# knelk/enerf

Hardware: AMD Instinct MI355X
Metric: train_rays_per_sec (higher is better)
Workload: dtype f32

## Files before the change

### enerf_amd/_lib.py

```python
import ctypes
import os

_HERE = os.path.dirname(os.path.abspath(__file__))
LIB_PATH = os.path.join(_HERE, "lib", "libenerf_hip.so")
if os.environ.get("ENERF_LIB_PATH"):
    LIB_PATH = os.environ["ENERF_LIB_PATH"]

_c = ctypes
_vp, _u32, _f32, _int, _sz = _c.c_void_p, _c.c_uint32, _c.c_float, _c.c_int, _c.c_size_t

SIGNATURES = {
    "enerf_near_far_from_aabb": [_vp, _vp, _vp, _u32, _f32, _vp, _vp, _vp],
    "enerf_polar_from_ray": [_vp, _vp, _f32, _u32, _vp, _vp],
    "enerf_morton3D": [_vp, _u32, _vp, _vp],
    "enerf_morton3D_invert": [_vp, _u32, _vp, _vp],
    "enerf_packbits": [_vp, _u32, _f32, _vp, _vp],
    "enerf_march_rays_train": [_vp, _vp, _vp, _f32, _f32, _u32, _u32, _u32, _u32, _u32, _vp, _vp, _vp, _vp, _vp,
                               _vp, _vp, _u32, _vp],
    "enerf_march_fuse_near_far": [_vp, _f32],
    "enerf_march_mirror_count": [_vp],
    "enerf_march_rays_train_ex": [_vp, _vp, _vp, _f32, _f32, _u32, _u32, _u32, _u32, _u32, _vp, _vp, _vp, _vp, _vp,
                                  _vp, _vp, _u32, _u32, _vp],
    "enerf_march_rays_train_count": [_vp, _vp, _vp, _f32, _f32, _u32, _u32, _u32, _u32, _vp, _vp, _vp, _vp, _u32, _u32,
                                     _vp],
# ... 31 lines not shown
    "enerf_mlp32_io16": [_int],
    "enerf_grid_adam_from_records_ex": [_vp, _vp, _vp, _vp, _vp, _u32, _u32, _f32, _f32, _f32, _f32, _u32, _u32, _vp, _vp,
                                        _vp, _vp, _vp, _vp, _vp, _vp],
    "enerf_grid_adam_from_records": [_vp, _vp, _vp, _vp, _vp, _u32, _u32, _f32, _f32, _f32, _f32, _u32, _vp],
    "enerf_sh_encode_forward": [_vp, _vp, _u32, _u32, _u32, _int, _vp, _int, _vp],
    "enerf_sh_encode_backward": [_vp, _vp, _u32, _u32, _u32, _vp, _vp, _int, _vp],
    "enerf_ffmlp_forward": [_vp, _vp, _u32, _u32, _u32, _u32, _u32, _u32, _u32, _vp, _vp, _int, _vp],
    "enerf_ffmlp_inference": [_vp, _vp, _u32, _u32, _u32, _u32, _u32, _u32, _u32, _vp, _vp, _int, _vp],
    "enerf_ffmlp_backward": [_vp, _vp, _vp, _vp, _u32, _u32, _u32, _u32, _u32, _u32, _u32, _int, _vp, _vp, _vp,
                             _int, _vp],
    "enerf_ffnerf_inference": [_vp, _vp, _vp, _vp, _u32, _int, _vp, _vp, _vp],
    "enerf_mlp32_forward": [_vp, _vp, _u32, _u32, _u32, _u32, _u32, _u32, _vp, _vp, _u32, _u32, _vp, _vp],
    "enerf_mlp32_forward_p": [_vp, _vp, _u32, _u32, _u32, _u32, _u32, _u32, _u32, _u32, _vp, _vp, _u32, _u32, _vp, _vp,
                              _vp],
    "enerf_mlp32_backward_p": [_vp, _vp, _vp, _vp, _u32, _u32, _u32, _vp, _u32, _u32, _u32, _u32, _u32, _vp, _vp, _u32,
                               _u32, _vp, _u32, _vp, _vp, _u32, _vp],
    "enerf_mlp32_forward_sh": [_vp, _vp, _u32, _u32, _u32, _u32, _u32, _u32, _vp, _vp, _u32, _u32, _vp, _vp, _vp],
    "enerf_mlp32_backward": [_vp, _vp, _vp, _vp, _u32, _u32, _u32, _u32, _u32, _vp, _vp, _vp, _u32, _u32, _vp, _u32, _vp, _vp,
                             _u32, _vp],
    "enerf_sh_encode_forward_strided": [_vp, _vp, _u32, _u32, _u32, _vp],
    "enerf_debug_grid_level_mask": [_u32],
    "enerf_debug_sweep_route": [_u32, _u32],
    "enerf_debug_sweep_schedule": [_u32, _u32, _u32, _vp, _u32],
    "enerf_debug_mlp32_wgrad_blocks": [_u32],
    "enerf_debug_mlp32_grid_caps": [_u32, _u32],
    "enerf_debug_march_wave_max_rays": [_u32],
    "enerf_debug_march_bg_blocks": [_u32],
    "enerf_debug_march_clip": [_int],
    "enerf_march_rays_use_box": [_int],
    "enerf_grid_owner_range": [ctypes.c_uint64, ctypes.c_uint64, _f32],
    "enerf_ffmlp_recompute": [_int],
    "enerf_amp_begin": [_vp, _vp, _vp, _vp],
    "enerf_amp_end": [_f32, _f32, _int, _vp],
    "enerf_amp_cancel": [],
    "enerf_debug_march_thread_min_rays": [_u32],
    "enerf_event_loss_fwd_bwd": [_vp, _vp, _vp, _u32, _u32, _u32, _f32, _f32, _f32, _vp, _vp, _vp, _vp, _vp],
    "enerf_event_pair_rays": [_vp, _vp, _vp, _vp, _u32, _vp, _vp, _u32, _u32, _vp, _vp, _vp, _vp, _u32, _f32, _f32, _f32,
                              _f32, _vp, _vp, _vp, _vp, _vp, _vp, _vp, _vp, _vp],
    "enerf_occupied_box_update": [_vp, _u32, _u32, _f32, _vp],
    "enerf_debug_mlp32_fused_backward": [_int],
    "enerf_mlp32_precision": [_int],
    "enerf_mlp32_recompute": [_int],
    "enerf_debug_grid_bwd_binned": [_u32, _u32],
    "enerf_density_grid_cells": [_vp, _u32, _u32, _f32, _u32, _c.c_uint64, _vp, _vp, _vp],
    "enerf_mark_untrained_grid": [_vp, _u32, _u32, _f32, _f32, _f32, _f32, _u32, _u32, _f32, _vp, _vp],
    "enerf_density_grid_update": [_vp, _vp, _u32, _u32, _u32, _f32, _f32, _f32, _vp, _vp, _vp, _u32, _vp, _vp],
# ... 206 lines not shown
```

### enerf_amd/csrc/common.h

```cpp
#pragma once
#include <hip/hip_runtime.h>
#include <stdint.h>
#include <stdio.h>

#include "../../include/enerf_hip.h"

namespace enerf {

constexpr int kWave = 64;

void set_error(const char* fmt, ...);

inline int check_hip(hipError_t e, const char* what) {
    if (e != hipSuccess) {
        set_error("%s: %s", what, hipGetErrorString(e));
        return (int)e;
    }
    return 0;
}

#define ENERF_BADARG(...)            \
    do {                             \
        enerf::set_error(__VA_ARGS__); \
        return ENERF_E_BADARG;       \
// ... 9 lines not shown
    int id;
    hipStream_t s;
    void* slot;
    bool ext;
    ProfScope(int kernel_id, hipStream_t stream, bool ext = false);
    ~ProfScope();
    hipEvent_t start() const;
    hipEvent_t stop() const;
    void units(double n) const;
};

struct AmpState {
    const float* scale;
    uint32_t* found_inf;
    const uint32_t* skipped;
};
AmpState amp_state();

void* workspace(int slot, size_t bytes);
uint64_t workspace_generation();
uint32_t num_cus();
int workspace_family_enter(int family, hipStream_t s);
int single_device_guard(const char* what);
enum { WS_SCAN = 0, WS_COMPACT = 1, WS_FFMLP = 2, WS_GRIDBWD = 3, WS_MARCH = 4, WS_DENSITY = 5, WS_MLP32_DEFER = 6, WS_AABB = 7, WS_AABB_CALL = 8, WS_FFMLP_W = 9, WS_NERF_FRAGS = 10, WS_NERF_PART = 11, WS_MARCH2 = 12, WS_SLOTS = 13 };

__host__ __device__ inline uint32_t div_up(uint32_t a, uint32_t b) { return (a + b - 1) / b; }

struct SplitJob {
    const float* src[5];
    const uint32_t* map;
    uint32_t* out;
    uint32_t threads;
};
struct ValidRows {
    const int32_t* count;
    uint32_t base, cap;
};
int grid_encode_forward(const float* inputs, const void* embeddings, const int32_t* offsets, void* outputs, uint32_t B,
                        uint32_t D, uint32_t C, uint32_t L, float S, uint32_t H, int calc_grad_inputs, void* dy_dx,
                        uint32_t gridtype, int dtype, int out_layout, float in_add, float in_mul, enerf_stream_t stream,
                        const ValidRows& grid_valid_rows, const SplitJob* job = nullptr, bool* carried = nullptr);
int grid_encode_backward(const void* grad, const float* inputs, const int32_t* offsets, void* grad_embeddings, uint32_t B,
                         uint32_t D, uint32_t C, uint32_t L, float S, uint32_t H, int calc_grad_inputs, const void* dy_dx,
                         void* grad_inputs, uint32_t gridtype, int dtype, int grad_layout, float in_add, float in_mul,
                         uint32_t flags, uint32_t reserve_B, enerf_stream_t stream, const ValidRows& grid_valid_rows);
struct MlpCall {
    ValidRows rows;
// ... 130 lines not shown
```

### enerf_amd/csrc/density_update.hip

```cpp

#include "common.h"
#include "sweep_points.h"

using namespace enerf;

namespace {

__device__ __forceinline__ uint32_t morton3(uint32_t x, uint32_t y, uint32_t z) { return sweep_morton3(x, y, z); }
__device__ __forceinline__ uint32_t compact_bits(uint32_t x) {
    x = x & 0x49249249;
    x = (x | (x >> 2)) & 0xc30c30c3;
    x = (x | (x >> 4)) & 0x0f00f00f;
    x = (x | (x >> 8)) & 0xff0000ff;
    x = (x | (x >> 16)) & 0x0000ffff;
    return x;
}

__global__ void __launch_bounds__(256) k_cells_full(Cascades cs, uint32_t C, uint32_t H, uint32_t logH, uint64_t seed,
                                                    int32_t* __restrict__ indices, float* __restrict__ xyzs) {
    const uint32_t H3 = H * H * H;
    const uint32_t p = blockIdx.x * blockDim.x + threadIdx.x;
    if (p >= C * H3) return;
    const uint32_t cas = p / H3, cell = p - cas * H3;
    const uint32_t x = cell & (H - 1), y = (cell >> logH) & (H - 1), z = cell >> (2 * logH);
// ... 197 lines not shown
    }
    __syncthreads();
    const uint32_t nh = heavy_n < 64u ? heavy_n : 64u;
    for (uint32_t e = 0; e < nh; e++) {
        const uint32_t key = heavy[e][0], c = heavy[e][1], at = heavy[e][2];
        for (uint32_t j = threadIdx.x; j < c; j += 256) out[at + j] = key;
    }
}

__global__ void __launch_bounds__(256) k_cells_from_keys(Cascades cs, uint32_t P, uint32_t H, uint32_t bits,
                                                         uint64_t seed, const uint32_t* __restrict__ keys,
                                                         int32_t* __restrict__ indices, float* __restrict__ xyzs) {
    const uint32_t p = blockIdx.x * blockDim.x + threadIdx.x;
    if (p >= P) return;
    const uint32_t key = keys[p];
    const uint32_t idx = key & ((1u << bits) - 1), cas = key >> bits;
    indices[p] = (int32_t)idx;
    cell_position(cs, cas, H, compact_bits(idx), compact_bits(idx >> 1), compact_bits(idx >> 2), rand4(seed, p),
                  xyzs + (size_t)p * 3);
}

__global__ void __launch_bounds__(256) k_tmp_scatter(const int32_t* __restrict__ indices, const float* __restrict__ sigmas,
                                                     uint32_t n_per_cas, uint32_t P, uint32_t H3, float scale,
                                                     float* __restrict__ tmp, uint32_t H, uint32_t logH) {
    const uint32_t p = blockIdx.x * blockDim.x + threadIdx.x;
    if (p >= P) return;
    const uint32_t cas = p / n_per_cas;
    uint32_t idx;
    if (indices) {
        idx = (uint32_t)indices[p];
    } else {
        const uint32_t cell = p - cas * n_per_cas;
        idx = morton3(cell & (H - 1), (cell >> logH) & (H - 1), cell >> (2 * logH));
    }
    tmp[(size_t)cas * H3 + idx] = sigmas[p] * scale;
}

constexpr uint32_t kSumSlots = 16, kSumStride = 16, kSumBytes = kSumSlots * kSumStride * 8;

__global__ void k_zero_sums(double* __restrict__ sum) { sum[threadIdx.x] = 0.0; }

__device__ __forceinline__ float ema1(float g, float t, float decay, float& acc) {
    if (g >= 0.0f && t >= 0.0f) g = fmaxf(g * decay, t);
    acc += fmaxf(g, 0.0f);
    return g;
}

__global__ void __launch_bounds__(256) k_ema_mean(float* __restrict__ grid, const float* __restrict__ tmp, uint32_t total4,
                                                  float decay, double* __restrict__ sum) {
    __shared__ float wsum[4];
    float acc = 0.0f;
    for (uint32_t i = blockIdx.x * blockDim.x + threadIdx.x; i < total4; i += gridDim.x * blockDim.x) {
        float4 g = reinterpret_cast<float4*>(grid)[i];
        const float4 t = reinterpret_cast<const float4*>(tmp)[i];
        g.x = ema1(g.x, t.x, decay, acc); g.y = ema1(g.y, t.y, decay, acc);
        g.z = ema1(g.z, t.z, decay, acc); g.w = ema1(g.w, t.w, decay, acc);
        reinterpret_cast<float4*>(grid)[i] = g;
    }
    for (int o = 32; o > 0; o >>= 1) acc += __shfl_down(acc, o, 64);
    if (lane_id() == 0) wsum[threadIdx.x >> 6] = acc;
    __syncthreads();
    if (threadIdx.x == 0)
        atomicAdd(sum + (blockIdx.x % kSumSlots) * kSumStride, (double)((wsum[0] + wsum[1]) + (wsum[2] + wsum[3])));
}

__global__ void __launch_bounds__(256) k_packbits_mean(const float* __restrict__ grid, uint32_t nbytes,
                                                       const double* __restrict__ sum, double inv_total,
                                                       float density_thresh, uint8_t* __restrict__ bitfield,
                                                       const int32_t* __restrict__ step_counter, uint32_t total_step,
                                                       double* __restrict__ stats) {
    double total = 0.0;
    for (uint32_t k = 0; k < kSumSlots; k++) total += sum[k * kSumStride];
    const float mean = (float)(total * inv_total);
    const float thresh = fminf(mean, density_thresh);
    const uint32_t n = blockIdx.x * blockDim.x + threadIdx.x;
    if (n == 0) {
        stats[0] = (double)mean;
        long long c = 0;
        for (uint32_t s = 0; s < total_step; s++) c += step_counter[s * 2];
        stats[1] = (double)c;
    }
    if (n >= nbytes) return;
    const float4 a = reinterpret_cast<const float4*>(grid)[(size_t)n * 2];
    const float4 b = reinterpret_cast<const float4*>(grid)[(size_t)n * 2 + 1];
    uint32_t bits = 0;
    bits |= a.x > thresh ? 1u : 0u;  bits |= a.y > thresh ? 2u : 0u;
    bits |= a.z > thresh ? 4u : 0u;  bits |= a.w > thresh ? 8u : 0u;
    bits |= b.x > thresh ? 16u : 0u; bits |= b.y > thresh ? 32u : 0u;
    bits |= b.z > thresh ? 64u : 0u; bits |= b.w > thresh ? 128u : 0u;
    bitfield[n] = (uint8_t)bits;
}

__global__ void __launch_bounds__(256) k_mark_untrained(const float* __restrict__ poses, uint32_t n_poses,
                                                        uint32_t pose_stride, float tan_x, float tan_y, Cascades cs,
                                                        uint32_t C, uint32_t H, float* __restrict__ grid) {
    const uint32_t H3 = H * H * H;
    const uint32_t p = blockIdx.x * blockDim.x + threadIdx.x;
    if (p >= C * H3) return;
    const uint32_t cas = p / H3, idx = p - cas * H3;
// ... 85 lines not shown
                              float cy, uint32_t C, uint32_t H, float bound, float* density_grid,
                              enerf_stream_t stream) {
    if (!grid_shape_ok(C, H)) ENERF_BADARG("mark_untrained_grid: C=%u H=%u", C, H);
    if (pose_stride != 16 && pose_stride != 12) ENERF_BADARG("mark_untrained_grid: poses are [B,4,4] or [B,3,4] fp32");
    if (fx == 0.0f || fy == 0.0f) ENERF_BADARG("mark_untrained_grid: zero focal length");
    const uint32_t cells = C * H * H * H;
    k_mark_untrained<<<div_up(cells, 256), 256, 0, (hipStream_t)stream>>>(poses, n_poses, pose_stride, cx / fx, cy / fy,
                                                                          make_cascades(C, H, bound), C, H,
                                                                          density_grid);
    ENERF_LAUNCH_CHECK("mark_untrained_grid");
    return 0;
}

int enerf_density_grid_update(const int32_t* indices, const float* sigmas, uint32_t n_per_cascade, uint32_t C, uint32_t H,
                              float sigma_scale, float decay, float density_thresh, float* density_grid,
                              uint8_t* bitfield, const int32_t* step_counter, uint32_t total_step, double* stats,
                              enerf_stream_t stream) {
    if (!grid_shape_ok(C, H)) ENERF_BADARG("density_grid_update: C=%u H=%u", C, H);
    if (total_step > 16) ENERF_BADARG("density_grid_update: total_step %u > 16", total_step);
    if (!stats) ENERF_BADARG("density_grid_update: stats is required");
    hipStream_t s = (hipStream_t)stream;
    const uint32_t H3 = H * H * H;
    const size_t cells = (size_t)C * H3;
    if (int ew = workspace_family_enter(1, s)) return ew;
    char* ws = (char*)workspace(WS_DENSITY, kSumBytes + cells * 4);
    if (!ws) return ENERF_E_NOMEM;
    double* sum = (double*)ws;
    float* tmp = (float*)(ws + kSumBytes);
    k_zero_sums<<<1, kSumSlots * kSumStride, 0, s>>>(sum);
    int e = check_hip(hipMemsetAsync(tmp, 0xFF, cells * 4, s), "density_grid_update: memset");
    if (e) return e;
    const uint32_t P = n_per_cascade * C;
    if (!indices && n_per_cascade != H3) ENERF_BADARG("density_grid_update: indices may be NULL for a full sweep only");
    if (P) k_tmp_scatter<<<div_up(P, 256), 256, 0, s>>>(indices, sigmas, n_per_cascade, P, H3, sigma_scale, tmp, H, log2u(H));
    k_ema_mean<<<2048, 256, 0, s>>>(density_grid, tmp, (uint32_t)(cells / 4), decay, sum);
    const uint32_t nbytes = (uint32_t)(cells / 8);
    k_packbits_mean<<<div_up(nbytes, 256), 256, 0, s>>>(density_grid, nbytes, sum, 1.0 / (double)cells, density_thresh,
                                                        bitfield, step_counter, total_step, stats);
    ENERF_LAUNCH_CHECK("density_grid_update");
    return 0;
}

}
```

### enerf_amd/csrc/gridencoder.hip

```cpp
#include <hip/hip_ext.h>
#include <hip/hip_fp16.h>
#include <math.h>

#include <type_traits>
#include <utility>

#include "common.h"
#include "sweep_points.h"

using namespace enerf;

namespace {

#ifdef ENERF_TA_TIMING
__device__ uint32_t g_ta_log[4 * 4096];
__device__ uint32_t g_ta_wg[2 * 2048];
__device__ unsigned long long g_ta_marks[8];
#define TA_MARK_IN(k) do { if (blockIdx.x == 0 && threadIdx.x == 0) g_ta_marks[k] = __builtin_amdgcn_s_memrealtime(); } while (0)
#define TA_MARK_OUT(k) do { if (threadIdx.x == 0) atomicMax(&g_ta_marks[k], (unsigned long long)__builtin_amdgcn_s_memrealtime()); } while (0)
__device__ unsigned long long g_bin_ph[32 * 8];
#define BIN_PH(k) do { if (threadIdx.x == 0) { const unsigned long long t_ = __builtin_amdgcn_s_memrealtime(); atomicAdd(&g_bin_ph[bin_lv * 8 + (k)], t_ - bin_t); bin_t = t_; } } while (0)
#else
#define TA_MARK_IN(k)
#define TA_MARK_OUT(k)
// ... 474 lines not shown
    }
    float q[3], in[3];
    sweep_point(gen, b, q);
    bool oob = false;
#pragma unroll
    for (int d = 0; d < 3; d++) {
        in[d] = (q[d] + tab.in_add) * tab.in_mul;
        oob |= (in[d] < 0 || in[d] > 1);
    }
    Feat<float, C>* out = outs + (out_layout == 0 ? (size_t)level * B + b
                                                  : out_layout == 1 ? (size_t)b * L + level : (size_t)level * Bp + b);
    if (oob) {
        *out = z;
        return;
    }
    const uint32_t off0 = (uint32_t)offsets[level];
    const LevelGeom<3> geom = make_geom<3>(gridtype, (uint32_t)offsets[level + 1] - off0, tab.resolution[level]);
    float pos[3];
    uint32_t pos_grid[3];
    *out = interp_level<float, 3, C>(in, tab.scale[level], geom, reinterpret_cast<const Feat<float, C>*>(grid) + off0,
                                     pos, pos_grid);
}

constexpr uint32_t kWalkUnit = 0x80000000u;
constexpr uint32_t kMaxSweepSegs = 48;
struct SweepSched {
    uint32_t first[kGroups + 1];
    uint32_t unit[kMaxSweepSegs];
    uint32_t chunk0[kMaxSweepSegs];
    uint32_t kend[kMaxSweepSegs];
};

template <int C, int WALK>
__device__ __forceinline__ void sweep_walk_point(uint32_t b, const float* __restrict__ grid,
                                                 const int32_t* __restrict__ offsets, float* __restrict__ outputs,
                                                 uint32_t B, uint32_t L, const LevelTab& tab, uint32_t gridtype,
                                                 int out_layout, const SweepGen& gen) {
    const uint32_t Bp = (B + 31u) & ~31u;
    Feat<float, C> z;
#pragma unroll
    for (int c = 0; c < C; c++) z.v[c] = 0.0f;
    Feat<float, C>* outs = reinterpret_cast<Feat<float, C>*>(outputs);
    if (b >= B) {
        if (out_layout == 2 && b < Bp) {
#pragma unroll
            for (uint32_t level = 0; level < (uint32_t)WALK; level++)
                if (level < L && level_enabled(tab, level)) outs[(size_t)level * Bp + b] = z;
        }
        return;
    }
    float q[3], in[3];
    sweep_point(gen, b, q);
    bool oob = false;
#pragma unroll
    for (int d = 0; d < 3; d++) {
        in[d] = (q[d] + tab.in_add) * tab.in_mul;
        oob |= (in[d] < 0 || in[d] > 1);
    }
#pragma unroll
    for (uint32_t level = 0; level < (uint32_t)WALK; level++) {
        if (level >= L || !level_enabled(tab, level)) continue;
        Feat<float, C>* out = outs + (out_layout == 0 ? (size_t)level * B + b
                                                      : out_layout == 1 ? (size_t)b * L + level : (size_t)level * Bp + b);
        if (oob) {
            *out = z;
            continue;
        }
        const uint32_t off0 = (uint32_t)offsets[level];
        const LevelGeom<3> geom = make_geom<3>(gridtype, (uint32_t)offsets[level + 1] - off0, tab.resolution[level]);
        float pos[3];
        uint32_t pos_grid[3];
        *out = interp_level<float, 3, C>(in, tab.scale[level], geom,
                                         reinterpret_cast<const Feat<float, C>*>(grid) + off0, pos, pos_grid);
    }
}

template <int C, int WALK>
__global__ void __launch_bounds__(kPtsPerBlock) k_grid_fwd_sweep(const float* __restrict__ grid,
                                                                 const int32_t* __restrict__ offsets,
                                                                 float* __restrict__ outputs, uint32_t B, uint32_t L,
                                                                 LevelTab tab, uint32_t gridtype, int out_layout,
                                                                 SweepGen gen, SweepSched sch) {
    const uint32_t xcd = blockIdx.x & 7u, group = xcd / kGroupXcds;
    const uint32_t k = (blockIdx.x >> 3) * kGroupXcds + xcd % kGroupXcds;
    const uint32_t end = sch.first[group + 1];
    uint32_t s = sch.first[group], kbeg = 0;
    while (s < end && k >= sch.kend[s]) kbeg = sch.kend[s++];
    if (s >= end) return;
    const uint32_t b = (sch.chunk0[s] + (k - kbeg)) * kPtsPerBlock + threadIdx.x;
    const uint32_t unit = sch.unit[s];
    if (WALK > 0 && unit == kWalkUnit) {
        sweep_walk_point<C, WALK>(b, grid, offsets, outputs, B, L, tab, gridtype, out_layout, gen);
        return;
    }
    if (!level_enabled(tab, unit)) return;
    sweep_level_point<C>(unit, b, grid, offsets, outputs, B, L, tab, gridtype, out_layout, gen);
}

template <int C>
__device__ __forceinline__ void scatter_add(float* row, float w, const float (&g)[C]) {
#pragma unroll
    for (int c = 0; c < C; c++) atomicAdd(row + c, w * g[c]);
}
template <int C>
__device__ __forceinline__ void scatter_add(__half* row, float w, const float (&g)[C]) {
    if constexpr (C % 2 == 0) {
#pragma unroll
        for (int c = 0; c < C; c += 2) {
            const __half2 v = __halves2half2(__float2half(w * g[c]), __float2half(w * g[c + 1]));
            unsafeAtomicAdd(reinterpret_cast<__half2*>(row + c), v);
        }
    } else {
#pragma unroll
        for (int c = 0; c < C; c++) {
            __half* addr = row + c;
// ... 929 lines not shown
                 \
            hipExtLaunchKernelGGL(k_prof_mark, dim3(1), dim3(64), 0, s, nullptr, ev_start, 0);                     \
            hipExtLaunchKernelGGL((k_grid_fwd<T, D, CC>), dim3(nblocks + carry), dim3(kPtsPerBlock), 0, s, nullptr, \
                                  ev_stop, 0, inputs, emb, offsets, outputs, B, L, tab, calc, dy_dx, gridtype,     \
                                  layout, nchunks, gen, job, carry);                                               \
        }                                                                                                          \
        else                                                                                                       \
            k_grid_fwd<T, D, CC><<<nblocks + carry, kPtsPerBlock, 0, s>>>(inputs, emb, offsets, outputs, B, L, tab, calc, \
                                                                          dy_dx, gridtype, layout, nchunks, gen, job, carry); \
    } while (0)
    switch (C) {
        case 1: ENERF_GF(1); break;
        case 2: ENERF_GF(2); break;
        case 4: ENERF_GF(4); break;
        case 8: ENERF_GF(8); break;
        default: ENERF_BADARG("GridEncoding: C must be 1, 2, 4, or 8.");
    }
#undef ENERF_GF
    return 0;
}

const float kSweepLevelUs[16] = {264.2f, 256.0f, 258.0f, 264.2f, 259.3f, 273.3f, 277.9f, 328.9f,
                                 394.1f, 501.5f, 591.6f, 655.3f, 683.6f, 697.8f, 700.1f, 704.0f};
const float kSweepWalkUs[6] = {0.0f, 0.0f, 0.0f, 0.0f, 463.2f, 531.5f};
uint32_t g_sweep_route = 0;
uint32_t g_sweep_walk = 5;

struct SweepSeg {
    uint32_t group, unit, chunk0, n;
};
int build_sweep_schedule(uint32_t L, uint32_t walk, uint32_t nchunks, SweepSeg* segs, uint32_t cap) {
    struct Unit {
        uint32_t id;
        double cost;
    };
    Unit units[kMaxLevels + 1];
    uint32_t nu = 0;
    const uint32_t walked = walk < L ? walk : L;
    if (walked) units[nu++] = {kWalkUnit, (double)kSweepWalkUs[walk] * walked / walk};
    for (uint32_t l = walked; l < L; l++) units[nu++] = {l, (double)kSweepLevelUs[l < 16 ? l : 15]};
    for (uint32_t i = 1; i < nu; i++)
        for (uint32_t j = i; j > 0 && units[j].cost > units[j - 1].cost; j--) std::swap(units[j], units[j - 1]);
    double total = 0.0;
    for (uint32_t i = 0; i < nu; i++) total += units[i].cost;
    const double target = total / kGroups;
    double load[kGroups] = {};
    SweepSeg raw[kMaxSweepSegs * 2];
    uint32_t nraw = 0;
    Unit pour[kMaxLevels + 1];
    uint32_t np = 0;
    for (uint32_t i = 0; i < nu; i++) {
        uint32_t g = 0;
        for (uint32_t h = 1; h < kGroups; h++)
            if (load[h] < load[g]) g = h;
        if (load[g] + units[i].cost <= target * (1.0 + 1e-6)) {
            raw[nraw++] = {g, units[i].id, 0u, nchunks};
            load[g] += units[i].cost;
        } else {
            pour[np++] = units[i];
        }
    }
    for (uint32_t i = 0; i < np; i++) {
        const double per_chunk = pour[i].cost / nchunks;
        uint32_t c0 = 0;
        while (c0 < nchunks) {
            uint32_t g = 0;
            for (uint32_t h = 1; h < kGroups; h++)
                if (load[h] < load[g]) g = h;
            const uint32_t left = nchunks - c0;
            const double want = (target - load[g]) / per_chunk;
            uint32_t n = want < 1.0 ? left : (uint32_t)fmin((double)left, floor(want + 0.5));
            if (n == 0) n = 1;
            if (left - n < 8u) n = left;
            if (nraw == kMaxSweepSegs * 2) return -1;
            raw[nraw++] = {g, pour[i].id, c0, n};
            load[g] += n * per_chunk;
            c0 += n;
        }
    }
    uint32_t ns = 0;
    for (uint32_t g = 0; g < kGroups; g++)
        for (uint32_t i = 0; i < nraw; i++) {
            if (raw[i].group != g) continue;
            if (ns == cap) return -1;
            segs[ns++] = raw[i];
        }
    return (int)ns;
}

int launch_sweep(const float* emb, const int32_t* offsets, float* outputs, uint32_t B, uint32_t C, uint32_t L,
                 const LevelTab& tab, uint32_t gridtype, int layout, const SweepGen& gen, hipStream_t s,
                 hipEvent_t ev_start, hipEvent_t ev_stop) {
    const uint32_t nchunks = div_up(layout == 2 ? ((B + 31u) & ~31u) : B, kPtsPerBlock);
    const uint32_t walk = g_sweep_walk;
    SweepSeg segs[kMaxSweepSegs];
    const int ns = build_sweep_schedule(L, walk, nchunks, segs, kMaxSweepSegs);
    if (ns < 0) ENERF_BADARG("grid_encode_forward_sweep: no schedule of %u levels within %u segments", L, kMaxSweepSegs);
    SweepSched sch{};
    uint32_t most = 0;
    for (uint32_t g = 0, i = 0; g < kGroups; g++) {
        sch.first[g] = i;
        uint32_t k = 0;
        for (; i < (uint32_t)ns && segs[i].group == g; i++) {
            sch.unit[i] = segs[i].unit;
            sch.chunk0[i] = segs[i].chunk0;
            sch.kend[i] = (k += segs[i].n);
        }
        sch.first[g + 1] = i;
        most = k > most ? k : most;
    }
    const uint32_t nblocks = 8u * div_up(most, kGroupXcds);
#define ENERF_GS(CC, WW)                                                                                            \
    do {                                                                                                            \
        if (ev_start) {                                                            \
            hipExtLaunchKernelGGL(k_prof_mark, dim3(1), dim3(64), 0, s, nullptr, ev_start, 0);                      \
            hipExtLaunchKernelGGL((k_grid_fwd_sweep<CC, WW>), dim3(nblocks), dim3(kPtsPerBlock), 0, s, nullptr,     \
                                  ev_stop, 0, emb, offsets, outputs, B, L, tab, gridtype, layout, gen, sch);        \
        } else                                                                                                      \
            k_grid_fwd_sweep<CC, WW><<<nblocks, kPtsPerBlock, 0, s>>>(emb, offsets, outputs, B, L, tab, gridtype,  \
                                                                      layout, gen, sch);                            \
    } while (0)
#define ENERF_GS_C(CC)                                                                                              \
    do {                                                                                                            \
        if (walk == 4) ENERF_GS(CC, 4);                                                                             \
        else if (walk == 5) ENERF_GS(CC, 5);                                                                        \
        else ENERF_GS(CC, 0);                                                                                       \
    } while (0)
    switch (C) {
        case 1: ENERF_GS_C(1); break;
        case 2: ENERF_GS_C(2); break;
        case 4: ENERF_GS_C(4); break;
        case 8: ENERF_GS_C(8); break;
        default: ENERF_BADARG("GridEncoding: C must be 1, 2, 4, or 8.");
    }
#undef ENERF_GS_C
#undef ENERF_GS
    return 0;
}

struct PendingRecords {
    uint32_t region = 0, L = 0, C = 0, D = 0, min_tiles = 0;
};
static PendingRecords g_pending;
static size_t g_own_lo = 0, g_own_hi = 0;
static float g_own_scale = 1.0f;
static uint32_t* g_overflow = nullptr;
static uint32_t g_session = 0;

static uint32_t* overflow_counter() {
    if (!g_overflow) {
        if (hipMalloc((void**)&g_overflow, 2 * sizeof(uint32_t)) != hipSuccess) return nullptr;
        if (hipMemset(g_overflow, 0, 2 * sizeof(uint32_t)) != hipSuccess) return nullptr;
    }
// ... 60 lines not shown
        if (calc)                                                                                                \
            k_grid_input_bwd<T, D, CC><<<div_up(B * D, 256), 256, 0, s>>>(grad, dy_dx, grad_inputs, B, L, layout); \
    } while (0)
    switch (C) {
        case 1: ENERF_GB(1); break;
        case 2: ENERF_GB(2); break;
        case 4: ENERF_GB(4); break;
        case 8: ENERF_GB(8); break;
        default: ENERF_BADARG("GridEncoding: C must be 1, 2, 4, or 8.");
    }
#undef ENERF_GB
    return 0;
}

}

extern "C" {

int enerf_debug_grid_level_mask(uint32_t mask) {
    g_level_mask = mask;
    return 0;
}

int enerf_debug_sweep_route(uint32_t route, uint32_t walk) {
    if (route > 1 || (walk != 0 && walk != 4 && walk != 5)) ENERF_BADARG("debug_sweep_route: route %u walk %u", route, walk);
    g_sweep_route = route;
    g_sweep_walk = walk;
    return 0;
}

int enerf_debug_sweep_schedule(uint32_t L, uint32_t walk, uint32_t nchunks, uint32_t* out, uint32_t cap) {
    if (L == 0 || L > kMaxLevels || nchunks == 0 || (walk != 0 && walk != 4 && walk != 5)) return -1;
    SweepSeg segs[kMaxSweepSegs];
    const int ns = build_sweep_schedule(L, walk, nchunks, segs, cap < kMaxSweepSegs ? cap : kMaxSweepSegs);
    for (int i = 0; i < ns; i++) {
        out[4 * i + 0] = segs[i].group;
        out[4 * i + 1] = segs[i].unit;
        out[4 * i + 2] = segs[i].chunk0;
        out[4 * i + 3] = segs[i].n;
    }
    return ns;
}

int enerf_debug_grid_bwd_binned(uint32_t min_batch, uint32_t min_tiles) {
    g_binned_min_batch = min_batch;
    g_binned_min_tiles = min_tiles ? min_tiles : 1u;
    return 0;
}

int enerf_grid_encode_forward(const float* inputs, const void* embeddings, const int32_t* offsets, void* outputs,
                              uint32_t B, uint32_t D, uint32_t C, uint32_t L, float S, uint32_t H, int calc_grad_inputs,
                              void* dy_dx, uint32_t gridtype, int dtype, int out_layout, float in_add, float in_mul,
                              enerf_stream_t stream) {
    return enerf::grid_encode_forward(inputs, embeddings, offsets, outputs, B, D, C, L, S, H, calc_grad_inputs, dy_dx, gridtype,
                                      dtype, out_layout, in_add, in_mul, stream, ValidRows{nullptr, 0, 0});
}

}

int enerf::grid_encode_forward(const float* inputs, const void* embeddings, const int32_t* offsets, void* outputs, uint32_t B,
                               uint32_t D, uint32_t C, uint32_t L, float S, uint32_t H, int calc_grad_inputs, void* dy_dx,
                               uint32_t gridtype, int dtype, int out_layout, float in_add, float in_mul, enerf_stream_t stream,
                               const ValidRows& grid_valid_rows, const SplitJob* job, bool* carried) {
    if (carried) *carried = false;
// ... 238 lines not shown
```

### include/enerf_hip.h

```cpp
#ifndef ENERF_HIP_H
#define ENERF_HIP_H

#include <stddef.h>
#include <stdint.h>

#ifdef __cplusplus
extern "C" {
#endif

typedef void* enerf_stream_t;

#define ENERF_OK 0
#define ENERF_E_BADARG (-1)
#define ENERF_E_NOMEM (-2)
#define ENERF_E_UNSUPPORTED (-3)

#define ENERF_F32 0
#define ENERF_F16 1
#define ENERF_BF16 2

const char* enerf_last_error(void);
#define ENERF_ABI_VERSION 6
int enerf_abi_version(void);
uint64_t enerf_workspace_generation(void);


int enerf_near_far_from_aabb(const float* rays_o, const float* rays_d, const float* aabb, uint32_t N,
                             float min_near, float* nears, float* fars, enerf_stream_t stream);

int enerf_polar_from_ray(const float* rays_o, const float* rays_d, float radius, uint32_t N, float* coords,
                         enerf_stream_t stream);

int enerf_morton3D(const int32_t* coords, uint32_t N, int32_t* indices, enerf_stream_t stream);

int enerf_morton3D_invert(const int32_t* indices, uint32_t N, int32_t* coords, enerf_stream_t stream);

int enerf_packbits(const float* grid, uint32_t N, float density_thresh, uint8_t* bitfield, enerf_stream_t stream);

int enerf_density_grid_cells(const float* density_grid, uint32_t C, uint32_t H, float bound, uint32_t n_uniform,
                             uint64_t seed, int32_t* indices, float* xyzs, enerf_stream_t stream);

int enerf_mark_untrained_grid(const float* poses, uint32_t n_poses, uint32_t pose_stride, float fx, float fy, float cx,
                              float cy, uint32_t C, uint32_t H, float bound, float* density_grid,
                              enerf_stream_t stream);

// ... 292 lines not shown
    float* const* dwseg_c;
    uint32_t nh_s, nh_c, w0_cols_c, out_c;
    const float* aabb;
    const uint8_t* bitfield;
    float min_near, dt_gamma;
    uint32_t cascade, grid_size, max_steps, perturb, march_flags, reserved0;
    float *table, *table_grad, *table_m, *table_v;
    float lr, beta1, beta2, eps;
    uint32_t table_step, n_small;
    float* const* small_p;
    const float* const* small_g;
    float* const* small_m;
    float* const* small_v;
    const uint32_t* small_n;
    const float* small_lr;
    const uint32_t* small_step;
    uint32_t flags, reserved;
    float *m_feats, *m_h32, *m_fb_s, *m_fb_c, *m_sigma, *m_rgb, *m_g_sigmas, *m_g_rgbs, *m_dx32, *m_dfeat;
} enerf_event_step_args;
int enerf_train_step_events(const enerf_event_step_args* args);

int enerf_debug_grid_level_mask(uint32_t mask);
int enerf_debug_sweep_route(uint32_t route, uint32_t walk);
int enerf_debug_sweep_schedule(uint32_t L, uint32_t walk, uint32_t nchunks, uint32_t* out, uint32_t cap);
int enerf_debug_grid_bwd_binned(uint32_t min_batch, uint32_t min_tiles);

#define ENERF_K_GRID_FWD 0
#define ENERF_K_GRID_BWD 1
#define ENERF_K_MARCH_TRAIN 2
#define ENERF_K_COMPOSITE_FWD 3
#define ENERF_K_COMPOSITE_BWD 4
#define ENERF_K_SH_FWD 5
#define ENERF_K_FFMLP_FWD 6
#define ENERF_K_FFMLP_BWD 7
#define ENERF_K_MARCH_INFER 8
#define ENERF_K_COMPOSITE_INFER 9
#define ENERF_K_TABLE_ADAM 10
#define ENERF_K_MLP_REDUCE 11
#define ENERF_K_COUNT 12

int enerf_march_train_samples(uint64_t* total, int reset, enerf_stream_t stream);
int enerf_prof_enable(int on);
int enerf_prof_enable_mask(uint32_t mask);
int enerf_prof_reset(void);
int enerf_prof_sample_every(uint32_t n);
int enerf_prof_read_units(int kernel_id, double* units, uint64_t* calls_seen);
int enerf_prof_read(int kernel_id, double* total_ms, uint64_t* launches);
// ... 59 lines not shown
```

Baseline: 11.91 million.

## Fuse full-sweep density EMA gather and widen grid-encode sweep walk levels

Density grid update on a full sweep no longer memsets and scatters into a temp buffer. k_ema_mean now gathers sigmas directly by de-interleaving Morton order, and the sum buffer is double-buffered so per-call zeroing is skipped after the first call. Separately, the grid-encode forward sweep gains a second walk unit and a default walk depth of 8 levels for C=2, with new cost tables for scheduling. The trade-off is non-coalesced float2 gathers in the EMA pass and more register-heavy walk kernels.

```diff
diff --git a/enerf_amd/_lib.py b/enerf_amd/_lib.py
--- a/enerf_amd/_lib.py
+++ b/enerf_amd/_lib.py
@@ -77,6 +77,10 @@
     "enerf_debug_grid_level_mask": [_u32],
     "enerf_debug_sweep_route": [_u32, _u32],
     "enerf_debug_sweep_schedule": [_u32, _u32, _u32, _vp, _u32],
+    "enerf_debug_sweep_route_ex": [_u32, _u32, _u32],
+    "enerf_debug_sweep_schedule_ex": [_u32, _u32, _u32, _u32, _vp, _u32],
+    "enerf_debug_sweep_costs": [_vp, _vp],
+    "enerf_debug_sweep_walk_costs": [_vp],
     "enerf_debug_mlp32_wgrad_blocks": [_u32],
     "enerf_debug_mlp32_grid_caps": [_u32, _u32],
     "enerf_debug_march_wave_max_rays": [_u32],
diff --git a/enerf_amd/csrc/common.h b/enerf_amd/csrc/common.h
--- a/enerf_amd/csrc/common.h
+++ b/enerf_amd/csrc/common.h
@@ -55,7 +55,7 @@
 uint32_t num_cus();
 int workspace_family_enter(int family, hipStream_t s);
 int single_device_guard(const char* what);
-enum { WS_SCAN = 0, WS_COMPACT = 1, WS_FFMLP = 2, WS_GRIDBWD = 3, WS_MARCH = 4, WS_DENSITY = 5, WS_MLP32_DEFER = 6, WS_AABB = 7, WS_AABB_CALL = 8, WS_FFMLP_W = 9, WS_NERF_FRAGS = 10, WS_NERF_PART = 11, WS_MARCH2 = 12, WS_SLOTS = 13 };
+enum { WS_SCAN = 0, WS_COMPACT = 1, WS_FFMLP = 2, WS_GRIDBWD = 3, WS_MARCH = 4, WS_DENSITY = 5, WS_MLP32_DEFER = 6, WS_AABB = 7, WS_AABB_CALL = 8, WS_FFMLP_W = 9, WS_NERF_FRAGS = 10, WS_NERF_PART = 11, WS_MARCH2 = 12, WS_DENSITY_SUMS = 13, WS_SLOTS = 14 };
 
 __host__ __device__ inline uint32_t div_up(uint32_t a, uint32_t b) { return (a + b - 1) / b; }
 
diff --git a/enerf_amd/csrc/density_update.hip b/enerf_amd/csrc/density_update.hip
--- a/enerf_amd/csrc/density_update.hip
+++ b/enerf_amd/csrc/density_update.hip
@@ -243,23 +243,26 @@
 
 __global__ void __launch_bounds__(256) k_tmp_scatter(const int32_t* __restrict__ indices, const float* __restrict__ sigmas,
                                                      uint32_t n_per_cas, uint32_t P, uint32_t H3, float scale,
-                                                     float* __restrict__ tmp, uint32_t H, uint32_t logH) {
+                                                     float* __restrict__ tmp) {
     const uint32_t p = blockIdx.x * blockDim.x + threadIdx.x;
     if (p >= P) return;
     const uint32_t cas = p / n_per_cas;
-    uint32_t idx;
-    if (indices) {
-        idx = (uint32_t)indices[p];
-    } else {
-        const uint32_t cell = p - cas * n_per_cas;
-        idx = morton3(cell & (H - 1), (cell >> logH) & (H - 1), cell >> (2 * logH));
-    }
-    tmp[(size_t)cas * H3 + idx] = sigmas[p] * scale;
-}
-
-constexpr uint32_t kSumSlots = 16, kSumStride = 16, kSumBytes = kSumSlots * kSumStride * 8;
-
-__global__ void k_zero_sums(double* __restrict__ sum) { sum[threadIdx.x] = 0.0; }
+    tmp[(size_t)cas * H3 + (uint32_t)indices[p]] = sigmas[p] * scale;
+}
+
+constexpr uint32_t kSumSlots = 16, kSumStride = 16, kSumSet = kSumSlots * kSumStride;
+struct SumState {
+    double sum[2][kSumSet];
+    uint32_t turn[2];
+};
+
+static_assert(kSumSet == 256, "one thread of a 256-thread workgroup per slot word (k_zero_sums, k_ema_mean)");
+
+__global__ void k_zero_sums(SumState* __restrict__ st) {
+    st->sum[0][threadIdx.x] = 0.0;
+    st->sum[1][threadIdx.x] = 0.0;
+    if (threadIdx.x < 2) st->turn[threadIdx.x] = 0;
+}
 
 __device__ __forceinline__ float ema1(float g, float t, float decay, float& acc) {
     if (g >= 0.0f && t >= 0.0f) g = fmaxf(g * decay, t);
@@ -267,13 +270,29 @@
     return g;
 }
 
-__global__ void __launch_bounds__(256) k_ema_mean(float* __restrict__ grid, const float* __restrict__ tmp, uint32_t total4,
-                                                  float decay, double* __restrict__ sum) {
+template <bool SWEEP>
+__global__ void __launch_bounds__(256) k_ema_mean(float* __restrict__ grid, const float* __restrict__ src, uint32_t total4,
+                                                  float decay, float scale, uint32_t logH, SumState* __restrict__ st) {
     __shared__ float wsum[4];
+    const uint32_t set = st->turn[0] & 1u;
+    if (blockIdx.x == 0) {
+        st->sum[set ^ 1u][threadIdx.x] = 0.0;
+        if (threadIdx.x == 0) st->turn[1] = set;
+    }
     float acc = 0.0f;
     for (uint32_t i = blockIdx.x * blockDim.x + threadIdx.x; i < total4; i += gridDim.x * blockDim.x) {
         float4 g = reinterpret_cast<float4*>(grid)[i];
-        const float4 t = reinterpret_cast<const float4*>(tmp)[i];
+        float4 t;
+        if constexpr (SWEEP) {
+            const uint32_t e = i * 4u, m = e & ((1u << (3 * logH)) - 1u);
+            const uint32_t cell = compact_bits(m) | compact_bits(m >> 1) << logH | compact_bits(m >> 2) << (2 * logH);
+            const float* row = src + (size_t)(e - m) + cell;
+            const float2 a = *reinterpret_cast<const float2*>(row);
+            const float2 b = *reinterpret_cast<const float2*>(row + (1u << logH));
+            t = make_float4(a.x * scale, a.y * scale, b.x * scale, b.y * scale);
+        } else {
+            t = reinterpret_cast<const float4*>(src)[i];
+        }
         g.x = ema1(g.x, t.x, decay, acc); g.y = ema1(g.y, t.y, decay, acc);
         g.z = ema1(g.z, t.z, decay, acc); g.w = ema1(g.w, t.w, decay, acc);
         reinterpret_cast<float4*>(grid)[i] = g;
@@ -282,20 +301,22 @@
     if (lane_id() == 0) wsum[threadIdx.x >> 6] = acc;
     __syncthreads();
     if (threadIdx.x == 0)
-        atomicAdd(sum + (blockIdx.x % kSumSlots) * kSumStride, (double)((wsum[0] + wsum[1]) + (wsum[2] + wsum[3])));
+        atomicAdd(&st->sum[set][(blockIdx.x % kSumSlots) * kSumStride], (double)((wsum[0] + wsum[1]) + (wsum[2] + wsum[3])));
 }
 
 __global__ void __launch_bounds__(256) k_packbits_mean(const float* __restrict__ grid, uint32_t nbytes,
-                                                       const double* __restrict__ sum, double inv_total,
+                                                       SumState* __restrict__ st, double inv_total,
                                                        float density_thresh, uint8_t* __restrict__ bitfield,
                                                        const int32_t* __restrict__ step_counter, uint32_t total_step,
                                                        double* __restrict__ stats) {
+    const uint32_t set = st->turn[1] & 1u;
     double total = 0.0;
-    for (uint32_t k = 0; k < kSumSlots; k++) total += sum[k * kSumStride];
+    for (uint32_t k = 0; k < kSumSlots; k++) total += st->sum[set][k * kSumStride];
     const float mean = (float)(total * inv_total);
     const float thresh = fminf(mean, density_thresh);
     const uint32_t n = blockIdx.x * blockDim.x + threadIdx.x;
     if (n == 0) {
+        st->turn[0] = set ^ 1u;
         stats[0] = (double)mean;
         long long c = 0;
         for (uint32_t s = 0; s < total_step; s++) c += step_counter[s * 2];
@@ -427,20 +448,31 @@
     hipStream_t s = (hipStream_t)stream;
     const uint32_t H3 = H * H * H;
     const size_t cells = (size_t)C * H3;
-    if (int ew = workspace_family_enter(1, s)) return ew;
-    char* ws = (char*)workspace(WS_DENSITY, kSumBytes + cells * 4);
-    if (!ws) return ENERF_E_NOMEM;
-    double* sum = (double*)ws;
-    float* tmp = (float*)(ws + kSumBytes);
-    k_zero_sums<<<1, kSumSlots * kSumStride, 0, s>>>(sum);
-    int e = check_hip(hipMemsetAsync(tmp, 0xFF, cells * 4, s), "density_grid_update: memset");
-    if (e) return e;
     const uint32_t P = n_per_cascade * C;
     if (!indices && n_per_cascade != H3) ENERF_BADARG("density_grid_update: indices may be NULL for a full sweep only");
-    if (P) k_tmp_scatter<<<div_up(P, 256), 256, 0, s>>>(indices, sigmas, n_per_cascade, P, H3, sigma_scale, tmp, H, log2u(H));
-    k_ema_mean<<<2048, 256, 0, s>>>(density_grid, tmp, (uint32_t)(cells / 4), decay, sum);
+    if (int ew = workspace_family_enter(1, s)) return ew;
+    SumState* st = (SumState*)workspace(WS_DENSITY_SUMS, sizeof(SumState));
+    if (!st) return ENERF_E_NOMEM;
+    static SumState* zeroed[16] = {};
+    int dev = 0;
+    if (hipGetDevice(&dev) != hipSuccess || dev < 0 || dev >= 16) dev = 0;
+    if (zeroed[dev] != st) {
+        k_zero_sums<<<1, kSumSet, 0, s>>>(st);
+        zeroed[dev] = st;
+    }
+    const uint32_t total4 = (uint32_t)(cells / 4), logH = log2u(H);
+    if (!indices) {
+        k_ema_mean<true><<<2048, 256, 0, s>>>(density_grid, sigmas, total4, decay, sigma_scale, logH, st);
+    } else {
+        float* tmp = (float*)workspace(WS_DENSITY, cells * 4);
+        if (!tmp) return ENERF_E_NOMEM;
+        int e = check_hip(hipMemsetAsync(tmp, 0xFF, cells * 4, s), "density_grid_update: memset");
+        if (e) return e;
+        if (P) k_tmp_scatter<<<div_up(P, 256), 256, 0, s>>>(indices, sigmas, n_per_cascade, P, H3, sigma_scale, tmp);
+        k_ema_mean<false><<<2048, 256, 0, s>>>(density_grid, tmp, total4, decay, sigma_scale, logH, st);
+    }
     const uint32_t nbytes = (uint32_t)(cells / 8);
-    k_packbits_mean<<<div_up(nbytes, 256), 256, 0, s>>>(density_grid, nbytes, sum, 1.0 / (double)cells, density_thresh,
+    k_packbits_mean<<<div_up(nbytes, 256), 256, 0, s>>>(density_grid, nbytes, st, 1.0 / (double)cells, density_thresh,
                                                         bitfield, step_counter, total_step, stats);
     ENERF_LAUNCH_CHECK("density_grid_update");
     return 0;
diff --git a/enerf_amd/csrc/gridencoder.hip b/enerf_amd/csrc/gridencoder.hip
--- a/enerf_amd/csrc/gridencoder.hip
+++ b/enerf_amd/csrc/gridencoder.hip
@@ -520,7 +520,7 @@
                                      pos, pos_grid);
 }
 
-constexpr uint32_t kWalkUnit = 0x80000000u;
+constexpr uint32_t kWalkUnit = 0x80000000u, kWalkUnit2 = 0x80000001u;
 constexpr uint32_t kMaxSweepSegs = 48;
 struct SweepSched {
     uint32_t first[kGroups + 1];
@@ -529,7 +529,7 @@
     uint32_t kend[kMaxSweepSegs];
 };
 
-template <int C, int WALK>
+template <int C, int LO, int HI>
 __device__ __forceinline__ void sweep_walk_point(uint32_t b, const float* __restrict__ grid,
                                                  const int32_t* __restrict__ offsets, float* __restrict__ outputs,
                                                  uint32_t B, uint32_t L, const LevelTab& tab, uint32_t gridtype,
@@ -542,7 +542,7 @@
     if (b >= B) {
         if (out_layout == 2 && b < Bp) {
 #pragma unroll
-            for (uint32_t level = 0; level < (uint32_t)WALK; level++)
+            for (uint32_t level = (uint32_t)LO; level < (uint32_t)HI; level++)
                 if (level < L && level_enabled(tab, level)) outs[(size_t)level * Bp + b] = z;
         }
         return;
@@ -556,7 +556,7 @@
         oob |= (in[d] < 0 || in[d] > 1);
     }
 #pragma unroll
-    for (uint32_t level = 0; level < (uint32_t)WALK; level++) {
+    for (uint32_t level = (uint32_t)LO; level < (uint32_t)HI; level++) {
         if (level >= L || !level_enabled(tab, level)) continue;
         Feat<float, C>* out = outs + (out_layout == 0 ? (size_t)level * B + b
                                                       : out_layout == 1 ? (size_t)b * L + level : (size_t)level * Bp + b);
@@ -573,7 +573,7 @@
     }
 }
 
-template <int C, int WALK>
+template <int C, int WALK, int WALK2>
 __global__ void __launch_bounds__(kPtsPerBlock) k_grid_fwd_sweep(const float* __restrict__ grid,
                                                                  const int32_t* __restrict__ offsets,
                                                                  float* __restrict__ outputs, uint32_t B, uint32_t L,
@@ -588,7 +588,11 @@
     const uint32_t b = (sch.chunk0[s] + (k - kbeg)) * kPtsPerBlock + threadIdx.x;
     const uint32_t unit = sch.unit[s];
     if (WALK > 0 && unit == kWalkUnit) {
-        sweep_walk_point<C, WALK>(b, grid, offsets, outputs, B, L, tab, gridtype, out_layout, gen);
+        sweep_walk_point<C, 0, WALK>(b, grid, offsets, outputs, B, L, tab, gridtype, out_layout, gen);
+        return;
+    }
+    if (WALK2 > WALK && unit == kWalkUnit2) {
+        sweep_walk_point<C, WALK, WALK2>(b, grid, offsets, outputs, B, L, tab, gridtype, out_layout, gen);
         return;
     }
     if (!level_enabled(tab, unit)) return;
@@ -1564,23 +1568,34 @@
 
 const float kSweepLevelUs[16] = {264.2f, 256.0f, 258.0f, 264.2f, 259.3f, 273.3f, 277.9f, 328.9f,
                                  394.1f, 501.5f, 591.6f, 655.3f, 683.6f, 697.8f, 700.1f, 704.0f};
-const float kSweepWalkUs[6] = {0.0f, 0.0f, 0.0f, 0.0f, 463.2f, 531.5f};
+constexpr uint32_t kMaxWalk = 9, kSplitWalk = 5;
+const float kSweepWalkUs[kMaxWalk + 1] = {0.0f, 0.0f, 0.0f, 0.0f, 463.2f, 531.5f, 611.2f, 704.5f, 825.4f, 1045.2f};
+const float kSweepWalk2Us[kMaxWalk + 1] = {0.0f, 0.0f, 0.0f, 0.0f, 0.0f, 0.0f, 0.0f, 421.7f, 648.3f, 813.2f};
+float g_sweep_walk_try[2 * (kMaxWalk + 1)];
+const float *g_sweep_walk_us = kSweepWalkUs, *g_sweep_walk2_us = kSweepWalk2Us;
 uint32_t g_sweep_route = 0;
-uint32_t g_sweep_walk = 5;
+uint32_t g_sweep_walk = 8;
+uint32_t g_sweep_walk2 = 8;
+
+bool sweep_walk_ok(uint32_t walk, uint32_t walk2) {
+    if (walk2 == walk) return walk == 0 || (walk >= 4 && walk <= kMaxWalk);
+    return walk == kSplitWalk && walk2 >= 7 && walk2 <= kMaxWalk;
+}
 
 struct SweepSeg {
     uint32_t group, unit, chunk0, n;
 };
-int build_sweep_schedule(uint32_t L, uint32_t walk, uint32_t nchunks, SweepSeg* segs, uint32_t cap) {
+int build_sweep_schedule(uint32_t L, uint32_t walk, uint32_t walk2, uint32_t nchunks, SweepSeg* segs, uint32_t cap) {
     struct Unit {
         uint32_t id;
         double cost;
     };
-    Unit units[kMaxLevels + 1];
+    Unit units[kMaxLevels + 2];
     uint32_t nu = 0;
-    const uint32_t walked = walk < L ? walk : L;
-    if (walked) units[nu++] = {kWalkUnit, (double)kSweepWalkUs[walk] * walked / walk};
-    for (uint32_t l = walked; l < L; l++) units[nu++] = {l, (double)kSweepLevelUs[l < 16 ? l : 15]};
+    const uint32_t walked = walk < L ? walk : L, walked2 = walk2 < L ? walk2 : L;
+    if (walked) units[nu++] = {kWalkUnit, (double)g_sweep_walk_us[walk] * walked / walk};
+    if (walked2 > walked) units[nu++] = {kWalkUnit2, (double)g_sweep_walk2_us[walk2] * (walked2 - walked) / (walk2 - walk)};
+    for (uint32_t l = walked2; l < L; l++) units[nu++] = {l, (double)kSweepLevelUs[l < 16 ? l : 15]};
     for (uint32_t i = 1; i < nu; i++)
         for (uint32_t j = i; j > 0 && units[j].cost > units[j - 1].cost; j--) std::swap(units[j], units[j - 1]);
     double total = 0.0;
@@ -1589,7 +1604,7 @@
     double load[kGroups] = {};
     SweepSeg raw[kMaxSweepSegs * 2];
     uint32_t nraw = 0;
-    Unit pour[kMaxLevels + 1];
+    Unit pour[kMaxLevels + 2];
     uint32_t np = 0;
     for (uint32_t i = 0; i < nu; i++) {
         uint32_t g = 0;
@@ -1634,9 +1649,10 @@
                  const LevelTab& tab, uint32_t gridtype, int layout, const SweepGen& gen, hipStream_t s,
                  hipEvent_t ev_start, hipEvent_t ev_stop) {
     const uint32_t nchunks = div_up(layout == 2 ? ((B + 31u) & ~31u) : B, kPtsPerBlock);
-    const uint32_t walk = g_sweep_walk;
+    uint32_t walk = g_sweep_walk, walk2 = g_sweep_walk2;
+    if (C != 2 && walk2 > kSplitWalk) walk = walk2 = kSplitWalk;
     SweepSeg segs[kMaxSweepSegs];
-    const int ns = build_sweep_schedule(L, walk, nchunks, segs, kMaxSweepSegs);
+    const int ns = build_sweep_schedule(L, walk, walk2, nchunks, segs, kMaxSweepSegs);
     if (ns < 0) ENERF_BADARG("grid_encode_forward_sweep: no schedule of %u levels within %u segments", L, kMaxSweepSegs);
     SweepSched sch{};
     uint32_t most = 0;
@@ -1652,25 +1668,34 @@
         most = k > most ? k : most;
     }
     const uint32_t nblocks = 8u * div_up(most, kGroupXcds);
-#define ENERF_GS(CC, WW)                                                                                            \
+#define ENERF_GS(CC, WW, W2)                                                                                          \
     do {                                                                                                            \
         if (ev_start) {                                                            \
             hipExtLaunchKernelGGL(k_prof_mark, dim3(1), dim3(64), 0, s, nullptr, ev_start, 0);                      \
-            hipExtLaunchKernelGGL((k_grid_fwd_sweep<CC, WW>), dim3(nblocks), dim3(kPtsPerBlock), 0, s, nullptr,     \
+            hipExtLaunchKernelGGL((k_grid_fwd_sweep<CC, WW, W2>), dim3(nblocks), dim3(kPtsPerBlock), 0, s, nullptr, \
                                   ev_stop, 0, emb, offsets, outputs, B, L, tab, gridtype, layout, gen, sch);        \
         } else                                                                                                      \
-            k_grid_fwd_sweep<CC, WW><<<nblocks, kPtsPerBlock, 0, s>>>(emb, offsets, outputs, B, L, tab, gridtype,  \
-                                                                      layout, gen, sch);                            \
+            k_grid_fwd_sweep<CC, WW, W2><<<nblocks, kPtsPerBlock, 0, s>>>(emb, offsets, outputs, B, L, tab,        \
+                                                                          gridtype, layout, gen, sch);              \
     } while (0)
 #define ENERF_GS_C(CC)                                                                                              \
     do {                                                                                                            \
-        if (walk == 4) ENERF_GS(CC, 4);                                                                             \
-        else if (walk == 5) ENERF_GS(CC, 5);                                                                        \
-        else ENERF_GS(CC, 0);                                                                                       \
+        if (walk == 4) ENERF_GS(CC, 4, 4);                                                                          \
+        else if (walk == 5) ENERF_GS(CC, 5, 5);                                                                     \
+        else ENERF_GS(CC, 0, 0);                                                                                    \
     } while (0)
     switch (C) {
         case 1: ENERF_GS_C(1); break;
-        case 2: ENERF_GS_C(2); break;
+        case 2:
+            if (walk == 5 && walk2 == 7) ENERF_GS(2, 5, 7);
+            else if (walk == 5 && walk2 == 8) ENERF_GS(2, 5, 8);
+            else if (walk == 5 && walk2 == 9) ENERF_GS(2, 5, 9);
+            else if (walk == 6) ENERF_GS(2, 6, 6);
+            else if (walk == 7) ENERF_GS(2, 7, 7);
+            else if (walk == 8) ENERF_GS(2, 8, 8);
+            else if (walk == 9) ENERF_GS(2, 9, 9);
+            else ENERF_GS_C(2);
+            break;
         case 4: ENERF_GS_C(4); break;
         case 8: ENERF_GS_C(8); break;
         default: ENERF_BADARG("GridEncoding: C must be 1, 2, 4, or 8.");
@@ -1777,17 +1802,45 @@
     return 0;
 }
 
-int enerf_debug_sweep_route(uint32_t route, uint32_t walk) {
-    if (route > 1 || (walk != 0 && walk != 4 && walk != 5)) ENERF_BADARG("debug_sweep_route: route %u walk %u", route, walk);
+int enerf_debug_sweep_route_ex(uint32_t route, uint32_t walk, uint32_t walk2) {
+    if (route > 1 || !sweep_walk_ok(walk, walk2))
+        ENERF_BADARG("debug_sweep_route: route %u walk %u walk2 %u", route, walk, walk2);
     g_sweep_route = route;
     g_sweep_walk = walk;
+    g_sweep_walk2 = walk2;
     return 0;
 }
-
-int enerf_debug_sweep_schedule(uint32_t L, uint32_t walk, uint32_t nchunks, uint32_t* out, uint32_t cap) {
-    if (L == 0 || L > kMaxLevels || nchunks == 0 || (walk != 0 && walk != 4 && walk != 5)) return -1;
+int enerf_debug_sweep_route(uint32_t route, uint32_t walk) { return enerf_debug_sweep_route_ex(route, walk, walk); }
+
+int enerf_debug_sweep_costs(float* level_us, float* walk_us) {
+    for (uint32_t i = 0; i < 16; i++) level_us[i] = kSweepLevelUs[i];
+    for (uint32_t i = 0; i <= kMaxWalk; i++) {
+        walk_us[i] = g_sweep_walk_us[i];
+        walk_us[10 + i] = g_sweep_walk2_us[i];
+    }
+    return 0;
+}
+
+int enerf_debug_sweep_walk_costs(const float* walk_us) {
+    if (!walk_us) {
+        g_sweep_walk_us = kSweepWalkUs;
+        g_sweep_walk2_us = kSweepWalk2Us;
+        return 0;
+    }
+    for (uint32_t i = 0; i <= kMaxWalk; i++) {
+        g_sweep_walk_try[i] = walk_us[i];
+        g_sweep_walk_try[kMaxWalk + 1 + i] = walk_us[10 + i];
+    }
+    g_sweep_walk_us = g_sweep_walk_try;
+    g_sweep_walk2_us = g_sweep_walk_try + kMaxWalk + 1;
+    return 0;
+}
+
+int enerf_debug_sweep_schedule_ex(uint32_t L, uint32_t walk, uint32_t walk2, uint32_t nchunks, uint32_t* out,
+                                  uint32_t cap) {
+    if (L == 0 || L > kMaxLevels || nchunks == 0 || !sweep_walk_ok(walk, walk2)) return -1;
     SweepSeg segs[kMaxSweepSegs];
-    const int ns = build_sweep_schedule(L, walk, nchunks, segs, cap < kMaxSweepSegs ? cap : kMaxSweepSegs);
+    const int ns = build_sweep_schedule(L, walk, walk2, nchunks, segs, cap < kMaxSweepSegs ? cap : kMaxSweepSegs);
     for (int i = 0; i < ns; i++) {
         out[4 * i + 0] = segs[i].group;
         out[4 * i + 1] = segs[i].unit;
@@ -1795,6 +1848,9 @@
         out[4 * i + 3] = segs[i].n;
     }
     return ns;
+}
+int enerf_debug_sweep_schedule(uint32_t L, uint32_t walk, uint32_t nchunks, uint32_t* out, uint32_t cap) {
+    return enerf_debug_sweep_schedule_ex(L, walk, walk, nchunks, out, cap);
 }
 
 int enerf_debug_grid_bwd_binned(uint32_t min_batch, uint32_t min_tiles) {
diff --git a/include/enerf_hip.h b/include/enerf_hip.h
--- a/include/enerf_hip.h
+++ b/include/enerf_hip.h
@@ -20,7 +20,7 @@
 #define ENERF_BF16 2
 
 const char* enerf_last_error(void);
-#define ENERF_ABI_VERSION 6
+#define ENERF_ABI_VERSION 7
 int enerf_abi_version(void);
 uint64_t enerf_workspace_generation(void);
 
@@ -359,7 +359,12 @@
 
 int enerf_debug_grid_level_mask(uint32_t mask);
 int enerf_debug_sweep_route(uint32_t route, uint32_t walk);
+int enerf_debug_sweep_route_ex(uint32_t route, uint32_t walk, uint32_t walk2);
 int enerf_debug_sweep_schedule(uint32_t L, uint32_t walk, uint32_t nchunks, uint32_t* out, uint32_t cap);
+int enerf_debug_sweep_schedule_ex(uint32_t L, uint32_t walk, uint32_t walk2, uint32_t nchunks, uint32_t* out,
+                                  uint32_t cap);
+int enerf_debug_sweep_costs(float* level_us, float* walk_us);
+int enerf_debug_sweep_walk_costs(const float* walk_us);
 int enerf_debug_grid_bwd_binned(uint32_t min_batch, uint32_t min_tiles);
 
 #define ENERF_K_GRID_FWD 0
```

Result: no change. 11.96 million, median of 4 (+0.4%).
